# xguo7/SND-VAE

Hardware: AMD Instinct MI355X
Metric: training graphs/sec + ELBO-step ms, N=4096 d=64, at 1/2/4/8 MI355X (higher is better)
Workload: dtype bf16; 1 GPU; C2: node-latent SND-VAE train step, N=4096, d=64, 8 graphs/GPU, HIP-graph replay; n_nodes=4096, latent=64, graphs_per_gpu=8, global_batch=8, parallelism=dp1, hip_graph=True

## Files before the change

snd_vae_amd/csrc/snd_elem.hip:

```cpp
#include "snd_elem.hpp"

#include <algorithm>
#include "snd_gemm.hpp"
#include "snd_tref.hpp"

namespace snd {
namespace {

template <typename T>
__device__ __forceinline__ T block_sum(T v) {
  __shared__ T sh[16];
  v = (sizeof(T) == 8) ? (T)wave_sum_d((double)v) : (T)wave_sum((float)v);
  const int w = threadIdx.x >> 6, nw = blockDim.x >> 6;
  if ((threadIdx.x & 63) == 0) sh[w] = v;
  __syncthreads();
  T t = 0;
  if (threadIdx.x == 0)
    for (int k = 0; k < nw; ++k) t += sh[k];
  return t;
}

constexpr int kReparamGrid = 2048;

__global__ void __launch_bounds__(256) reparam_fwd_kernel(ReparamFwdArgs a) {
// ... 290 lines not shown
  }
  sg = lane_rows_sum<CP>(sg, red);
  sb = lane_rows_sum<CP>(sb, red);
  if (threadIdx.x < width) {
    const int stride = (a.has_enc ? 2 * a.wenc : 0) + 2 * a.h;
    float* pp = a.part + (long long)blockIdx.x * stride;
    int o = 0;
    if (a.has_enc) {
      pp[c] = sge * kBnC;
      pp[a.wenc + c] = sbe;
      o = 2 * a.wenc;
    }
    if (c < a.h) {
      pp[o + c] = sg * kBnC;
      pp[o + a.h + c] = sb;
    }
  }
}

#ifndef SND_RED_PL
#define SND_RED_PL 2
#endif
#ifndef SND_RED_PLS
#define SND_RED_PLS 4
#endif
#ifndef SND_RED_PLW
#define SND_RED_PLW 2
#endif
constexpr long long kRedWide = 2048;
__host__ __device__ __forceinline__ int red_pl(int nparts, long long items) {
  return nparts >= 1024 ? 64
                        : (nparts >= 256 ? 32 : (nparts >= 64 ? (items >= kRedWide ? SND_RED_PL : 8) : (items >= kRedWide ? SND_RED_PLW : SND_RED_PLS)));
}
struct ReducePack {
  ReduceDesc d[kMaxReduce];
  int bstart[kMaxReduce + 1];
};

template <int NTF> __device__ void finalize_block(const FinalizeArgs& a);

template <bool FIN, bool ADAM>
__global__ void __launch_bounds__(256) reduce_kernel(ReducePack pk, FinalizeArgs fin, ReduceAdam ra) {
  if constexpr (FIN) {
    if (blockIdx.x == 0) { finalize_block<256>(fin); return; }
  }
  const int bid = (int)blockIdx.x - (FIN ? 1 : 0);
  int di = 0;
#pragma unroll
  for (int i = 1; i < kMaxReduce; ++i) di += bid >= pk.bstart[i] ? 1 : 0;
  di = __builtin_amdgcn_readfirstlane(di);
  const ReduceDesc& d = pk.d[di];
  const int bx = bid - pk.bstart[di];
  const bool dad = ADAM && ((ra.mask >> di) & 1ull);
  float lrt = 0.f;
  if (dad) {
    const int st = *ra.stepn;
    lrt = (float)((double)ra.lr * sqrt(1.0 - pow((double)ra.b2, st)) / (1.0 - pow((double)ra.b1, st)));
  }
  __shared__ double red[256];
  const int rows = d.rows > 0 ? d.rows : 1;
  const long long items = (long long)rows * d.len;
  const int PL = red_pl(d.nparts, items);
  const int IPB = 256 / PL;
  const int it = threadIdx.x % IPB, pl = threadIdx.x / IPB;
  const long long j = (long long)bx * IPB + it;
  int r = 0, i = 0;
  double acc = 0.0;
  float pi = 0.f, mi = 0.f, vi = 0.f, prev = 0.f;
  if (j < items) {
    r = (int)(j / d.len);
    i = (int)(j - (long long)r * d.len);
    if (pl == 0) {
      const float* dst = d.dst + (long long)r * d.dst_rs + i;
      if (d.accumulate) prev = *dst;
      if constexpr (ADAM) {
        if (dad) {
          const long long k = dst - ra.gbase;
          pi = ra.p[k]; mi = ra.m[k]; vi = ra.v[k];
        }
      }
    }
    const float* src = d.src + (long long)r * d.src_rs + i;
    int p = pl;
    for (; p + 7 * PL < d.nparts; p += 8 * PL) {
      float v[8];
#pragma unroll
      for (int u = 0; u < 8; ++u) v[u] = src[(long long)(p + u * PL) * d.stride];
#pragma unroll
      for (int u = 0; u < 8; ++u) acc += (double)v[u];
    }
    for (; p + 3 * PL < d.nparts; p += 4 * PL) {
      const float v0 = src[(long long)p * d.stride];
      const float v1 = src[(long long)(p + PL) * d.stride];
      const float v2 = src[(long long)(p + 2 * PL) * d.stride];
      const float v3 = src[(long long)(p + 3 * PL) * d.stride];
      acc += (double)v0;
      acc += (double)v1;
      acc += (double)v2;
      acc += (double)v3;
    }
    for (; p < d.nparts; p += PL) acc += (double)src[(long long)p * d.stride];
  }
  red[threadIdx.x] = acc;
  __syncthreads();
  if (pl == 0 && j < items) {
    double t = 0.0;
    for (int q = 0; q < PL; ++q) t += red[q * IPB + it];
    float* dst = d.dst + (long long)r * d.dst_rs + i;
    float v = (float)(t * (double)d.scale);
    if (d.accumulate) v += prev;
    *dst = v;
    if constexpr (ADAM) {
      if (dad) {
        const long long k = dst - ra.gbase;
        adam_elem(pi, mi, vi, __fmul_rn(v, 1.f), ra.b1, ra.b2, ra.eps, lrt);
        ra.m[k] = mi;
// ... 145 lines not shown
  return 0;
}

int launch_enc_bwd(const EncBwdArgs& a, int rows, hipStream_t s) {
  const int width = a.has_enc ? a.wenc : a.h;
  if (width > 256) { set_error("enc_bwd: width %d > 256", width); return SND_ERR_ARG; }
  dim3 grid(col_blocks(rows));
  if (width <= 64) hipLaunchKernelGGL(enc_bwd_kernel<64>, grid, dim3(256), 0, s, a, rows);
  else if (width <= 128) hipLaunchKernelGGL(enc_bwd_kernel<128>, grid, dim3(256), 0, s, a, rows);
  else hipLaunchKernelGGL(enc_bwd_kernel<256>, grid, dim3(256), 0, s, a, rows);
  SND_LAUNCH_CHECK("enc_bwd_kernel");
  return 0;
}

int launch_reduce(const ReduceDesc* d, int n, hipStream_t s, const FinalizeArgs* fin,
                  const ReduceAdam* adam) {
  SND_CHECK_ARG(!adam || (n <= 64 && adam->gbase && adam->p && adam->m && adam->v && adam->stepn),
                "reduce: fused Adam needs <= 64 descriptors and its operands");
  for (int base = 0; base < n || (base == 0 && fin); base += kMaxReduce) {
    const bool last = base + kMaxReduce >= n;
    ReduceAdam ra{};
    if (adam) {
      ra = *adam;
      ra.mask = adam->mask >> base;
      if (n - base < 64) ra.mask &= (1ull << (n - base)) - 1;
    }
    const bool ad = ra.mask != 0;
    ReducePack pk{};
    const int cnt = n - base < kMaxReduce ? n - base : kMaxReduce;
    long long nb = 0;
    for (int i = 0; i < kMaxReduce; ++i) {
      pk.bstart[i] = (int)nb;
      if (i < cnt) {
        pk.d[i] = d[base + i];
        const long long items = (long long)(pk.d[i].rows > 0 ? pk.d[i].rows : 1) * pk.d[i].len;
        const int ipb = 256 / red_pl(pk.d[i].nparts, items);
        nb += (items + ipb - 1) / ipb;
      }
    }
    pk.bstart[kMaxReduce] = (int)nb;
    if (fin && last) {
      if (ad) hipLaunchKernelGGL((reduce_kernel<true, true>), dim3((unsigned)nb + 1), dim3(256), 0, s, pk, *fin, ra);
      else hipLaunchKernelGGL((reduce_kernel<true, false>), dim3((unsigned)nb + 1), dim3(256), 0, s, pk, *fin, ra);
    } else {
      if (nb == 0) continue;
      if (ad) hipLaunchKernelGGL((reduce_kernel<false, true>), dim3((unsigned)nb), dim3(256), 0, s, pk, FinalizeArgs{}, ra);
      else hipLaunchKernelGGL((reduce_kernel<false, false>), dim3((unsigned)nb), dim3(256), 0, s, pk, FinalizeArgs{}, ra);
    }
    SND_LAUNCH_CHECK("reduce_kernel");
  }
  return 0;
}

int launch_finalize(const FinalizeArgs& a, hipStream_t s) {
  hipLaunchKernelGGL(finalize_kernel, dim3(1), dim3(kFinT), 0, s, a);
  SND_LAUNCH_CHECK("finalize_kernel");
  return 0;
}

}

using namespace snd;

extern "C" int snd_reparam_kl_blocks(int rows, int latent) { return reparam_blocks(rows, latent); }
extern "C" int snd_sigmoid_mse_blocks(int rows) { return head_blocks(rows); }

extern "C" int snd_sigmoid_mse(const float* u, int ldu, int rows, int cin, const float* w,
// ... 64 lines not shown
```

snd_vae_amd/csrc/snd_fast.hip:

```cpp
#include "snd_fast.hpp"
#include "snd_gather.hpp"
#include "snd_pack.hpp"

#include <algorithm>

namespace snd {

namespace {

constexpr int NT = 256;

typedef short v4s __attribute__((ext_vector_type(4)));
typedef short v8s __attribute__((ext_vector_type(8)));
typedef __attribute__((address_space(3))) v4s lds_v4s;

__device__ __forceinline__ int swz(int row, int kp) {
  return kp >= 128 ? (row & 15) : (kp == 64 ? ((row >> 1) & 7) : 0);
}

__device__ __forceinline__ uint4 pack8(float4 lo, float4 hi) {
  bf16x8 v;
  v[0] = (__bf16)lo.x; v[1] = (__bf16)lo.y; v[2] = (__bf16)lo.z; v[3] = (__bf16)lo.w;
  v[4] = (__bf16)hi.x; v[5] = (__bf16)hi.y; v[6] = (__bf16)hi.z; v[7] = (__bf16)hi.w;
  return __builtin_bit_cast(uint4, v);
// ... 399 lines not shown
                                               int vlo, int vhi, int kp, __bf16* dst,
                                               const void* zero) {
  const int lane = threadIdx.x & 63, w = threadIdx.x >> 6;
  const int lk = log2kc(kp), kc = 1 << lk;
  const int npc = ((nrows << lk) + 63) >> 6;
  for (int j = w; j < npc; j += 4) {
    const int q = (j << 6) + lane;
    const int row = q >> lk, pc = q & (kc - 1);
    const int c = pc ^ trsw(row, kp);
    const int gr = base + row;
    const bool v = row < nrows && gr >= vlo && gr < vhi && 8 * c < K;
    const void* g = v ? (const void*)(src + (long long)gr * ld + 8 * c) : zero;
    glds16(g, reinterpret_cast<char*>(dst) + (j << 10));
  }
}

__device__ __forceinline__ int tr_off(int row, int col, int kp) {
  const int c = col >> 3;
  return row * kp + (((c ^ trsw(row, kp)) << 3) | (col & 4));
}

constexpr int WGT = 1024;

__device__ __forceinline__ int cdiv_d(int a, int b) { return (a + b - 1) / b; }

struct WgUnit { int sub, s0, s1, glo, ghi; };

__device__ __forceinline__ WgUnit wg_unit(const WgArgs& a, int sub, int s0, int c1) {
  const int send = min(c1, sub + kRcRows);
  WgUnit u;
  u.sub = sub; u.s0 = s0;
  if (a.T == 1) { u.glo = sub; u.ghi = send; u.s1 = send; }
  else {
    const int gs = (s0 / a.npg) * a.npg;
    u.glo = gs; u.ghi = min(a.R, gs + a.npg); u.s1 = min(send, u.ghi);
  }
  return u;
}

constexpr int kWgStampWords = 12;
__device__ __forceinline__ void wg_stamp(unsigned* ts, int i, bool on) {
  if (on && threadIdx.x == 0 && i < kWgStampWords) ts[i] = (unsigned)__builtin_amdgcn_s_memrealtime();
}

template <int NBO, int NPW = 1>
__device__ __forceinline__ void wgrad_body(const WgArgs& a, const int bx, const int by, __bf16* lds,
                                           unsigned* tsp = nullptr) {
  const bool stamp = tsp != nullptr;
  const int T = a.T, H = (T - 1) >> 1;
  const int XR = kRcRows + T - 1;
  const int kpx = a.K <= 32 ? 32 : (a.K <= 64 ? 64 : 128);
  const int kpy = a.N <= 32 ? 32 : (a.N <= 64 ? 64 : 128);
  const int xch = ((XR << log2kc(kpx)) + 63) & ~63;
  const int bufe = (xch << 3) + kRcRows * kpy;
  const int tid = threadIdx.x, lane = tid & 63, w = __builtin_amdgcn_readfirstlane(tid >> 6);
  const int li = lane & 15, lg = lane >> 4, tq = li >> 2, tp = li & 3;
  const __bf16* xg = reinterpret_cast<const __bf16*>(a.x);
  const __bf16* dg = reinterpret_cast<const __bf16*>(a.dy);
  const int c0 = bx * a.rows_per_wg, c1 = min(a.R, c0 + a.rows_per_wg);
  auto stage = [&](const WgUnit& u, int b) __attribute__((always_inline)) {
    if (kdbg(a.dbg) & 2) return;
    __bf16* xs = lds + b * bufe;
    __bf16* ds = xs + (xch << 3);
    const int lkx = log2kc(kpx), lky = log2kc(kpy);
    const int npx = xch >> 6, npy = (kRcRows << lky) >> 6;
    for (int j = w; j < npx + npy; j += WGT / 64) {
      const bool isx = j < npx;
      const int jj = isx ? j : j - npx;
      const int lk = isx ? lkx : lky, kp = isx ? kpx : kpy;
      const int q = (jj << 6) + lane;
      const int row = q >> lk, pc = q & ((1 << lk) - 1);
      const int c = pc ^ trsw(row, kp);
      const void* g = a.zero;
      if (isx) {
        const int gr = u.sub - H + row;
        if (row < XR && gr >= u.glo && gr < u.ghi && 8 * c < a.K) g = xg + (long long)gr * a.ldx + 8 * c;
      } else {
        const int gr = u.sub + row;
        if (gr >= u.s0 && gr < u.s1 && 8 * c < a.N) g = dg + (long long)gr * a.lddy + 8 * c;
      }
      glds16_async(g, reinterpret_cast<char*>(isx ? xs : ds) + (jj << 10));
    }
  };

  const WgUnit u0 = wg_unit(a, c0, c0, c1);
  if (c0 < c1) stage(u0, 0);
  const int cbn = (a.K + 15) >> 4;
  const int P = T * cbn;
  bool pvs[NPW];
  int ts[NPW], cbs[NPW];
#pragma unroll
  for (int i = 0; i < NPW; ++i) {
    const int wl = w + 16 * i, p = by * a.pairs_per_wg + wl;
    pvs[i] = wl < a.pairs_per_wg && p < P;
    ts[i] = pvs[i] ? p / cbn : 0;
    cbs[i] = pvs[i] ? p - ts[i] * cbn : 0;
  }
  const bool pv = pvs[0];

  f32x4 acc[NPW][NBO];
#pragma unroll
  for (int i = 0; i < NPW; ++i)
#pragma unroll
    for (int j = 0; j < NBO; ++j) acc[i][j] = f32x4{0.f, 0.f, 0.f, 0.f};

  const int rk0 = 8 * lg + tq;
  int xoff[NPW], xoff2[NPW];
#pragma unroll
  for (int i = 0; i < NPW; ++i) {
    xoff[i] = tr_off(rk0 + ts[i], 16 * cbs[i] + 4 * tp, kpx);
    xoff2[i] = tr_off(rk0 + ts[i] + 4, 16 * cbs[i] + 4 * tp, kpx);
  }
  if (kdbg(a.dbg) & 32) return;
  const int doff = rk0 * kpy;
  const int swd = trsw(rk0, kpy), tpl = (4 * tp) & 4, tph = tp >> 1;
  wg_stamp(tsp, 2, stamp);
  if (c0 < c1) {
    WgUnit u = u0;
    for (int k = 0;; ++k) {
      __builtin_amdgcn_s_waitcnt(0x0F70);
      __syncthreads();
      wg_stamp(tsp, 3 + k, stamp && k < 6);
      int nsub = u.sub, ns0 = u.s1;
      if (ns0 >= min(c1, u.sub + kRcRows)) { nsub = u.sub + kRcRows; ns0 = nsub; }
      const bool more = nsub < c1;
      WgUnit un{};
      if (more) { un = wg_unit(a, nsub, ns0, c1); stage(un, (k + 1) & 1); }
      const __bf16* xs = lds + (k & 1) * bufe;
      const __bf16* ds = xs + (xch << 3);
// ... 12 lines not shown
#pragma unroll
            for (int i = 0; i < NPW; ++i)
              if (i == 0 || pvs[i]) acc[i][ob] = __builtin_amdgcn_mfma_f32_16x16x32_bf16(af, bxv[i], acc[i][ob], 0, 0, 0);
          }
        }
      }
      if (!more) break;
      u = un;
    }
  }
  if (kdbg(a.dbg) & 8) return;
  const int sK = a.sK, sn4 = a.sn4;
#pragma unroll
  for (int i = 0; i < NPW; ++i) {
    const int k = 16 * cbs[i] + li;
    if (!pvs[i] || k >= a.K) continue;
    float* row = a.slab + (long long)bx * T * sK * sn4 + ((long long)ts[i] * sK + a.wk0 + k) * sn4 + a.wn0;
#pragma unroll
    for (int ob = 0; ob < NBO; ++ob) {
      const int n0 = 16 * ob + 4 * lg;
      if (n0 < a.N)
        *reinterpret_cast<float4*>(row + n0) =
            make_float4(acc[i][ob][0], acc[i][ob][1], acc[i][ob][2], acc[i][ob][3]);
    }
  }
}

template <int NBO>
__global__ void __launch_bounds__(WGT) wgrad_kernel(WgArgs a) {
  extern __shared__ __attribute__((aligned(16))) __bf16 lds[];
  wgrad_body<NBO>(a, blockIdx.x, blockIdx.y, lds);
}

struct WgMultiPack {
  WgArgs a[kMaxWgMulti];
  int start[kMaxWgMulti + 1];
  int nseg;
  int stamp_base;
};
static_assert(sizeof(WgMultiPack) <= 4096, "wgrad_multi: kernel arguments over 4 KB");

__global__ void __launch_bounds__(WGT) __attribute__((amdgpu_waves_per_eu(8, 8)))
wgrad_multi_kernel(WgMultiPack m) {
  extern __shared__ __attribute__((aligned(16))) __bf16 lds[];
  __shared__ unsigned tsl[kWgStampWords];
  const bool stamp = (kdbg(m.a[0].dbg) & (1 << 21)) && m.a[0].stamps;
  wg_stamp(tsl, 0, stamp);
  if (kdbg(m.a[0].dbg) & 1) return;
  const int bid = blockIdx.y * gridDim.x + blockIdx.x;
  int s = 0;
  if (gridDim.y > 1) {
    s = blockIdx.y;
  } else {
#pragma unroll
    for (int i = 1; i < kMaxWgMulti; ++i) s += (int)blockIdx.x >= m.start[i] ? 1 : 0;
  }
  s = __builtin_amdgcn_readfirstlane(s);
  const WgArgs a = m.a[s];
  const int local = gridDim.y > 1 ? (int)blockIdx.x : (int)blockIdx.x - m.start[s];
  const int gx = cdiv_d(a.R, a.rows_per_wg);
  const int bx = local % gx, by = local / gx;
  const bool two = a.pairs_per_wg > WGT / 64;
  if (kdbg(a.dbg) & 16) return;
  unsigned* ts = stamp ? tsl : nullptr;
  wg_stamp(ts, 1, stamp);
  switch ((a.N + 15) >> 4) {
    case 1: if (two) wgrad_body<1, 2>(a, bx, by, lds, ts); else wgrad_body<1>(a, bx, by, lds, ts); break;
    case 2: if (two) wgrad_body<2, 2>(a, bx, by, lds, ts); else wgrad_body<2>(a, bx, by, lds, ts); break;
    case 3: if (two) wgrad_body<3, 2>(a, bx, by, lds, ts); else wgrad_body<3>(a, bx, by, lds, ts); break;
    default: if (two) wgrad_body<4, 2>(a, bx, by, lds, ts); else wgrad_body<4>(a, bx, by, lds, ts); break;
  }
  if (stamp) {
    __syncthreads();
    if (threadIdx.x == 0) {
      unsigned* o = m.a[0].stamps + ((long long)m.stamp_base + bid) * kWgStampWords;
      for (int i = 0; i < 9; ++i) o[i] = tsl[i];
      o[9] = (unsigned)__builtin_amdgcn_s_memrealtime();
      o[10] = __builtin_amdgcn_s_getreg((31 << 11) | 4);
      o[11] = __builtin_amdgcn_s_getreg((31 << 11) | 20);
    }
  }
}

struct HeadFastPack { HeadFastArgs h[2]; };

template <int CIN, int COUT>
__device__ __forceinline__ void head_rows(const HeadFastArgs& h, int R) {
  constexpr int NQ = CIN * COUT + COUT + 3 * CIN;
  __shared__ float red[16][NQ];
  __shared__ double sred[4];
  const int tid = threadIdx.x, lane = tid & 63, w = tid >> 6;
  const int r = blockIdx.x * kHeadFastRows + tid;
  const bool rv = r < R;
  float wv[CIN][COUT], bv[COUT], gk[CIN], bk[CIN];
#pragma unroll
  for (int k = 0; k < CIN; ++k) {
#pragma unroll
    for (int o = 0; o < COUT; ++o) wv[k][o] = h.w[k * COUT + o];
    gk[k] = h.gamma[k] * kBnC;
    bk[k] = h.beta[k];
  }
#pragma unroll
  for (int o = 0; o < COUT; ++o) bv[o] = h.b[o];
  float u[CIN], yv[CIN];
#pragma unroll
  for (int k = 0; k < CIN; ++k) { u[k] = 0.f; yv[k] = 0.f; }
  if (rv) {
// ... 209 lines not shown
  SND_CHECK_ARG(a.ldx % 8 == 0 && a.ldo % 4 == 0, "rowconv: ldx %% 8 / ldo %% 4");
  a.npb = rc_cols_per_block(a.T, a.kp, a.np);
  SND_CHECK_ARG(a.npb > 0, "rowconv: LDS image too large (T %d kp %d np %d)", a.T, a.kp, a.np);
  for (;;) {
    const int nb = (int)round_up(cdiv(a.npb, 2), 16);
    if ((a.dbg & (1 << 19)) || a.g_rowptr || rc_blocks(a.R) * cdiv(a.np, a.npb) >= SND_RC_FILL || nb < 32 ||
        nb >= a.npb) break;
    a.npb = nb;
  }
  SND_CHECK_ARG(a.x && a.wpk && a.out && a.zero && a.x_bf16, "rowconv: null operand / fp32 x");
  SND_CHECK_ARG(!a.colpart || (a.ncp >= 1 && a.ncp <= 4), "rowconv: ncp");
  SND_CHECK_ARG(a.npg > 0, "rowconv: npg");
  SND_CHECK_ARG(!a.g_rowptr || (epi == RC_ENC0 && a.T == 1 && a.kp == 64 && a.K <= 64 && a.np <= 64 && a.g_colidx &&
                                a.gout && a.ldgo % 8 == 0 && a.ldx % 8 == 0 && a.npb == a.np),
                "rowconv: the gathered x rows need RC_ENC0, T 1, kp 64, one column window");
  switch (epi) {
    case RC_LIN: return rc_launch_epi<RC_LIN>(a, s);
    case RC_FWD:
      SND_CHECK_ARG(a.y && a.bias && a.gamma && a.beta && a.ldy % 4 == 0, "rowconv fwd: BN operands");
      return rc_launch_epi<RC_FWD>(a, s);
    case RC_DECBWD:
      SND_CHECK_ARG(a.y && a.gamma && a.beta && a.ldy % 4 == 0, "rowconv decbwd: BN operands");
      return rc_launch_epi<RC_DECBWD>(a, s);
    case RC_ENC1:
      SND_CHECK_ARG(a.p && a.xf && a.gamma && a.g2 && a.b2 && a.h % 4 == 0, "rowconv enc1 operands");
      return rc_launch_epi<RC_ENC1>(a, s);
    case RC_ENC0:
      SND_CHECK_ARG(a.p && a.w0 && a.gamma && a.f <= 4, "rowconv enc0 operands");
      return rc_launch_epi<RC_ENC0>(a, s);
    default: set_error("rowconv: bad epilogue %d", epi); return SND_ERR_ARG;
  }
}

static WgArgs wg_norm(const WgArgs& a) {
  WgArgs x = a;
  if (x.sK == 0) { x.sK = x.K; x.sn4 = wgrad_n4(x.N); x.wk0 = 0; x.wn0 = 0; }
  return x;
}

#ifndef SND_WG_SPLIT_LDS
#define SND_WG_SPLIT_LDS (80 * 1024)
#endif
constexpr size_t kWgSplitLds = SND_WG_SPLIT_LDS;
static int wg_split(const WgArgs& a, WgArgs* out, int cap) {
  const bool sk = a.K > 64 && wg_lds_bytes(a.T, a.K, std::min(a.N, 64)) > kWgSplitLds, sn = a.N > 64;
  int n = 0;
  for (int k0 = 0; k0 < a.K; k0 += sk ? 64 : a.K)
    for (int n0 = 0; n0 < a.N; n0 += sn ? 64 : a.N) {
      if (n >= cap) return -1;
      WgArgs w = a;
      w.K = sk ? std::min(64, a.K - k0) : a.K;
      w.N = sn ? std::min(64, a.N - n0) : a.N;
      w.x = static_cast<const __bf16*>(a.x) + k0;
      w.dy = static_cast<const __bf16*>(a.dy) + n0;
      w.wk0 = a.wk0 + k0; w.wn0 = a.wn0 + n0;
      w.pairs_per_wg = std::min(a.pairs_per_wg, a.T * cdiv(w.K, 16));
      out[n++] = w;
    }
  return n;
}

static int wg_multi_flush(WgMultiPack& pk, int total, size_t lds, hipStream_t s) {
  if (pk.nseg == 0) return 0;
  for (int i = pk.nseg; i <= kMaxWgMulti; ++i) pk.start[i] = total;
  bool uniform = pk.nseg > 1;
  for (int i = 1; i < pk.nseg; ++i) uniform = uniform && pk.start[i + 1] - pk.start[i] == pk.start[1];
  const dim3 grid = uniform ? dim3(pk.start[1], pk.nseg) : dim3(total);
  hipLaunchKernelGGL(wgrad_multi_kernel, grid, dim3(WGT), lds, s, pk);
  SND_LAUNCH_CHECK("wgrad_multi_kernel");
  return 0;
}

int launch_wgrad_multi(const WgArgs* a, int n, hipStream_t s) {
  if (n <= 0) return 0;
  WgMultiPack pk{};
  size_t lds = 0;
  int total = 0, base = 0;
  pk.nseg = 0;
  const bool stamps = a[0].stamps != nullptr;
  for (int i = 0; i < n; ++i) {
    const WgArgs x0 = wg_norm(a[i]);
    if (x0.R <= 0) continue;
    SND_CHECK_ARG(x0.T == 1 || x0.T == 5, "wgrad_multi: T must be 1 or 5");
    SND_CHECK_ARG(x0.K > 0 && x0.K <= 128 && x0.N > 0 && x0.N <= 128, "wgrad_multi: K %d N %d", x0.K, x0.N);
    SND_CHECK_ARG(x0.ldx % 8 == 0 && x0.lddy % 8 == 0 && x0.x_bf16 && x0.dy_bf16,
                  "wgrad_multi: bf16 operands with leading dims %% 8");
    SND_CHECK_ARG(x0.rows_per_wg % kRcRows == 0 && x0.pairs_per_wg >= 1 && x0.pairs_per_wg <= 2 * WGT / 64,
                  "wgrad_multi: geometry");
    SND_CHECK_ARG(x0.x && x0.dy && x0.slab && x0.zero && x0.npg > 0, "wgrad_multi: null operand");
    SND_CHECK_ARG(x0.sn4 % 4 == 0 && x0.wn0 % 4 == 0 && x0.wk0 + x0.K <= x0.sK &&
                  x0.wn0 + wgrad_n4(x0.N) <= x0.sn4, "wgrad_multi: slab window");
    WgArgs win[4];
    const int nw = wg_split(x0, win, 4);
    SND_CHECK_ARG(nw > 0, "wgrad_multi: window split");
    for (int j = 0; j < nw; ++j) {
      if (pk.nseg == kMaxWgMulti) {
        SND_TRY(wg_multi_flush(pk, total, lds, s));
        base += total;
        pk = WgMultiPack{};
        pk.stamp_base = base;
        lds = 0;
        total = 0;
      }
      const WgArgs& x = win[j];
      const int P = x.T * cdiv(x.K, 16);
      pk.a[pk.nseg] = x;
      pk.start[pk.nseg] = total;
      total += cdiv(x.R, x.rows_per_wg) * cdiv(P, x.pairs_per_wg);
      lds = std::max(lds, wg_lds_bytes(x.T, x.K, x.N));
      ++pk.nseg;
      SND_CHECK_ARG(!stamps || ((long long)base + total) * kWgStampWords <= a[0].stamp_words,
                    "wgrad_multi: %d workgroups' stamps exceed the %lld-word buffer", base + total,
                    a[0].stamp_words);
    }
  }
  return wg_multi_flush(pk, total, lds, s);
}

WgGeom wgrad_geom(int R, int T, int K, int N, int chunks) {
  WgGeom g{};
  const int P = T * cdiv(K, 16);
  g.pairs_per_wg = std::min(P, WGT / 64);
  g.gy = cdiv(P, g.pairs_per_wg);
  if (chunks > 0) {
    g.pairs_per_wg = std::min(P, 2 * WGT / 64);
    g.gy = cdiv(P, g.pairs_per_wg);
    g.rows_per_wg = (int)round_up(cdiv(R, chunks), kRcRows);
    g.gx = cdiv(R, g.rows_per_wg);
    return g;
  }
  int gx = std::max(1, 256 / g.gy);
  if ((long long)T * K * N >= 65536) gx = std::min(gx, 64);
  g.rows_per_wg = (int)round_up(cdiv(R, gx), kRcRows);
  g.gx = cdiv(R, g.rows_per_wg);
  return g;
}

int launch_wgrad(const WgArgs& a0, hipStream_t s) {
  const WgArgs a = wg_norm(a0);
  if (a.R <= 0) return 0;
  SND_CHECK_ARG(a.T == 1 || a.T == 5, "wgrad: T must be 1 or 5");
  SND_CHECK_ARG(a.K > 0 && a.K <= 128 && a.N > 0 && a.N <= 128, "wgrad: K %d N %d", a.K, a.N);
  SND_CHECK_ARG(a.ldx % 8 == 0 && a.lddy % 8 == 0 && a.x_bf16 && a.dy_bf16,
                "wgrad: bf16 operands with leading dims %% 8");
  SND_CHECK_ARG(a.rows_per_wg % kRcRows == 0 && a.pairs_per_wg >= 1 && a.pairs_per_wg <= WGT / 64,
                "wgrad: geometry");
  SND_CHECK_ARG(a.x && a.dy && a.slab && a.zero && a.npg > 0, "wgrad: null operand");
  const int P = a.T * cdiv(a.K, 16);
  dim3 grid(cdiv(a.R, a.rows_per_wg), cdiv(P, a.pairs_per_wg));
  switch (cdiv(a.N, 16)) {
    case 1: return wg_launch<1>(a, grid, s);
    case 2: return wg_launch<2>(a, grid, s);
    case 3: return wg_launch<3>(a, grid, s);
    case 4: return wg_launch<4>(a, grid, s);
    case 5: return wg_launch<5>(a, grid, s);
    case 6: return wg_launch<6>(a, grid, s);
    case 7: return wg_launch<7>(a, grid, s);
    default: return wg_launch<8>(a, grid, s);
  }
}

static thread_local int g_dbg = 0;
int debug_flags() { return g_dbg; }

static int fast_init_attributes_once() {
#define SND_ATTR(K)                                                                       \
  if (hipFuncSetAttribute(reinterpret_cast<const void*>(K),                               \
                          hipFuncAttributeMaxDynamicSharedMemorySize, (int)kMaxDynLds) != \
      hipSuccess) {                                                                       \
    set_error("hipFuncSetAttribute(%s) failed", #K);                                      \
    return SND_ERR_HIP;                                                                   \
  }
#define SND_ATTR4(E) SND_ATTR((rowconv_kernel<E, 1>)) SND_ATTR((rowconv_kernel<E, 2>)) \
                     SND_ATTR((rowconv_kernel<E, 3>)) SND_ATTR((rowconv_kernel<E, 4>))
  SND_ATTR4(RC_LIN) SND_ATTR4(RC_FWD) SND_ATTR4(RC_DECBWD) SND_ATTR4(RC_ENC1) SND_ATTR4(RC_ENC0)
#undef SND_ATTR4
  SND_ATTR((wgrad_kernel<1>)) SND_ATTR((wgrad_kernel<2>)) SND_ATTR((wgrad_kernel<3>))
  SND_ATTR((wgrad_kernel<4>)) SND_ATTR((wgrad_kernel<5>)) SND_ATTR((wgrad_kernel<6>))
  SND_ATTR((wgrad_kernel<7>)) SND_ATTR((wgrad_kernel<8>))
#undef SND_ATTR
  if (hipFuncSetAttribute(reinterpret_cast<const void*>(wgrad_multi_kernel),
                          hipFuncAttributeMaxDynamicSharedMemorySize, (int)kWgMultiLds) != hipSuccess) {
    set_error("hipFuncSetAttribute(wgrad_multi_kernel) failed");
    return SND_ERR_HIP;
  }
  return 0;
}

int fast_init_attributes() {
  static const int rc = fast_init_attributes_once();
  return rc;
}

}

extern "C" int snd_debug_set(int flags) {
  snd::g_dbg = flags;
  return 0;
}
```

snd_vae_amd/csrc/snd_fast.hpp:

```cpp
#pragma once
#include "snd_common.hpp"

namespace snd {

struct ColMap {
  int a, b, offb;
  __host__ __device__ int phys() const { return b ? offb + b : a; }
  __host__ __device__ bool valid(int c) const { return c < a || (b && c >= offb && c < offb + b); }
  __host__ __device__ int logical(int c) const { return c < a ? c : c - offb + a; }
};
inline ColMap colmap_plain(int n) { return {n, 0, n}; }
inline ColMap colmap_split(int a, int b) { return {a, b, (int)round_up(a, 8)}; }

struct PackSrc {
  const float* w;
  int A, B;
  int a0, a1, b0, b1;
  int n_off, k_off;
  int mode;
};
struct PackDesc {
  __bf16* dst;
  int T, kp, np;
  int nsrc;
  PackSrc s[2];
};
constexpr int kMaxPack = 16;
int launch_pack(const PackDesc* d, int n, hipStream_t s);
size_t pack_bytes(int T, int kp, int np);

enum RcEpi {
  RC_LIN = 0,
  RC_FWD = 1,
// ... 1 lines not shown
  RC_ENC1 = 3,
  RC_ENC0 = 4,
};
struct RcArgs {
  const void* x; int ldx; int K; int x_bf16;
  int R, npg, T;
  const __bf16* wpk; int kp, np;
  int N;
  ColMap cols;
  const float* bias; const float* gamma; const float* beta;
  const float* bias_b; const float* gamma_b; const float* beta_b;
  float* y; int ldy;
  void* out; int ldo; int out_bf16;
  float* colpart; int ncp;
  const float* p; int ldp;
  const float* xf; int ldxf; int f;
  const float* w0;
  const float* g2; const float* b2;
  int h;
  const void* zero;
  int dbg;
  int ktail; const float* wtail; int ldwt;
  int npb;
  const int* g_rowptr; const int* g_colidx; void* gout; int ldgo;
};
constexpr int kRcRows = 128;
constexpr size_t kRcLdsLimit = 136 * 1024;
int rc_blocks(int R);
size_t rc_lds_bytes(int T, int kp, int np);
int rc_cols_per_block(int T, int kp, int np);
int launch_rowconv(const RcArgs& a, int epi, hipStream_t s);

struct WgArgs {
  const void* x; int ldx; int K; int x_bf16;
  const void* dy; int lddy; int N; int dy_bf16;
  int R, npg, T;
  int rows_per_wg;
  int pairs_per_wg;
  float* slab;
  const void* zero;
  int dbg;
  int sK, sn4, wk0, wn0;
  unsigned* stamps;
  long long stamp_words;
};
struct WgGeom { int rows_per_wg, pairs_per_wg, gx, gy; };
WgGeom wgrad_geom(int R, int T, int K, int N, int chunks = 0);
inline int wgrad_n4(int N) { return (N + 3) & ~3; }
int launch_wgrad(const WgArgs& a, hipStream_t s);
constexpr int kMaxWgMulti = 32;
int launch_wgrad_multi(const WgArgs* a, int n, hipStream_t s);

struct HeadFastArgs {
  const void* u; int ldu; int u_bf16;
  const float* y; int ldy;
  const float* gamma; const float* beta;
  int cin;
  const float* w; const float* b; int cout;
  const float* target; int ldt;
  float count;
  float* yhat;
  __bf16* dy; int lddy;
  float* part;
  double* sse;
};
constexpr int kHeadFastRows = 256;
int heads_fast_blocks(int R);
bool heads_fast_supported(int cin, int cout);
int heads_fast_parts(int cin, int cout);
int launch_heads_fast(const HeadFastArgs* h, int n, int R, hipStream_t s);

struct Gcn0Args {
  const int* rowptr; const int* colidx; int R;
  const float* x; int ldx; int f;
  const float* w0; const float* g0; const float* b0; int h0;
  __bf16* h1; int ldh1;
  float* ax; __bf16* axb;
  int xcd_nbg;
  const int* row_order;
  PackDesc pack[kMaxPack]; int pack_blk[kMaxPack + 1]; int npack;
};
int xcd_nbg(int npg, int ngraphs);
int gcn0_blocks(int R);
int launch_gcn0(const Gcn0Args& a, hipStream_t s);
// ... 61 lines not shown
```

snd_vae_amd/csrc/snd_step.hip:

```cpp
#include <algorithm>
#include <cstdarg>
#include <cstdlib>
#include <cstring>
#include <new>
#include <string>
#include <vector>

#include "snd_dec.hpp"
#include "snd_decode.hpp"
#include "snd_elem.hpp"
#include "snd_fast.hpp"
#include "snd_gemm.hpp"
#include "snd_head.hpp"
#include "snd_spmm.hpp"
#include "snd_tref.hpp"
#include "snd_sg.hpp"
#include "snd_zzt.hpp"

namespace snd {

static thread_local char g_err[512] = "";

void set_error(const char* fmt, ...) {
  va_list ap;
// ... 1374 lines not shown
                 p.c.h1, SND_SPMM_PLAIN, (__bf16*)(ws + p.buf("FDXW1")), p.c.h1};
    a.xcd_nbg = xcd_nbg(p.N, p.B);
    use_tiles(a, batch, p.N, p.B);
    return launch_spmm_bf16(a, s);
  }
  if (!strncmp(kernel, "tref_", 5)) {
    SND_CHECK_ARG(p.tref && !p.sg && p.last_params, "snd_plan_launch: no graph-latent step has run");
    Ctx x{&p, ws, p.last_params, p.last_grads, s};
    const snd_config_t& c = p.c;
    const long long KH = (long long)p.N * p.W, CP = (long long)p.N * p.dj;
    const float adj_scale = (float)(2.0 * (double)c.norm / ((double)p.B * p.N * (double)p.N));
    const __bf16* gb = p.fast_enc ? reinterpret_cast<const __bf16*>(x.f("FG")) : nullptr;
    if (!strcmp(kernel, "tref_head_fwd")) {
      TrefHeadFwdArgs a{gb ? nullptr : x.f("G"), KH, p.B, x.w("enc.Wh"), c.g_hidden, x.w("enc.bh"),
                        x.f("PHF"), gb, p.ldg, p.W, p.N};
      return launch_tref_head_fwd(a, s);
    }
    if (!strcmp(kernel, "tref_head_bwd")) {
      TrefHeadBwdArgs a{gb ? nullptr : x.f("G"), KH, p.B, x.w("enc.Wh"), c.g_hidden, x.f("DH"),
                        x.g("enc.Wh"), gb ? nullptr : x.f("DG"), gb, p.ldg, p.W, p.N,
                        gb ? reinterpret_cast<__bf16*>(x.f("FDG")) : nullptr};
      return launch_tref_head_bwd(a, s);
    }
    if (!strcmp(kernel, "tref_proj_fwd")) {
      TrefProjFwdArgs a{x.f("ZL"), p.B, c.latent, x.w("dec.Wp"), x.w("dec.bp"), CP, x.f("Z")};
      return launch_tref_proj_fwd(a, s);
    }
    if (!strcmp(kernel, "tref_proj_bwd")) {
      TrefProjBwdArgs a{x.f("ZL"), p.B, c.latent, x.w("dec.Wp"), CP, x.f("DZDEC"), x.f("DJD"), x.f("EJ"),
                        adj_scale, x.g("dec.Wp"), x.g("dec.bp"), x.f("PDZ")};
      return launch_tref_proj_bwd(a, s);
    }
  }
  if (!strcmp(kernel, "wgrad_multi")) {
    SND_CHECK_ARG(!p.last_wq.empty(), "snd_plan_launch: no multi-segment weight-gradient launch yet");
    std::vector<WgArgs> q = p.last_wq;
    for (auto& w : q) {
      w.dbg = debug_flags();
      const bool st = (w.dbg & (1 << 21)) && p.dec_fused;
      w.stamps = st ? reinterpret_cast<unsigned*>(ws + p.buf("PDHS")) : nullptr;
      w.stamp_words = st ? p.buf_numel("PDHS") : 0;
    }
    return launch_wgrad_multi(q.data(), (int)q.size(), s);
  }
  if (!strcmp(kernel, "head_bwd")) {
    SND_CHECK_ARG(p.head_bwd && p.last_params, "snd_plan_launch: head_bwd needs a fused-head step first");
    Ctx x{&p, ws, p.last_params, p.last_grads, s};
    x.zts = p.last_zts;
    const double pairs = (double)p.B * p.N * (double)p.N;
    return head_bwd_fused(x, batch, (float)(2.0 * (double)p.c.norm / pairs),
                          (float)((double)p.c.beta / ((double)p.RH * p.c.latent)));
  }
  if (!strcmp(kernel, "head_fwd")) {
    SND_CHECK_ARG(p.head_fused && p.last_params, "snd_plan_launch: head_fwd needs a fused-head step first");
    Ctx x{&p, ws, p.last_params, p.last_grads, s};
    const ZztStage stg = zzt_stage(ws + p.buf("ZSTAGE"), p.B, p.N, p.dj, p.c.dtype);
    return head_fwd_fused(x, batch, nullptr, 0ull, nullptr, stg);
  }
  if (!strncmp(kernel, "dec:", 4) || !strcmp(kernel, "pack")) {
    SND_CHECK_ARG(p.fast && p.last_params, "snd_plan_launch: no fast-path step has run");
    SND_TRY(fast_init_attributes());
    Ctx x{&p, ws, p.last_params, p.last_grads, s};
    if (kernel[0] == 'p') return pack_decoder(x);
    if (!strcmp(kernel, "dec:fwd") || !strcmp(kernel, "dec:bwd")) {
      SND_CHECK_ARG(p.dec_fused, "snd_plan_launch: %s needs the fused decoder", kernel);
      return decoder_fast(x, batch, kernel[4] == 'f' ? 100 : 101);
    }
    return decoder_fast(x, batch, atoi(kernel + 4));
  }
  set_error("snd_plan_launch: unknown kernel '%s'", kernel);
  return SND_ERR_ARG;
}

void final_reduce_descs(const Ctx& x, std::vector<ReduceDesc>& rd) {
// ... 405 lines not shown
```

Baseline: 39340 graphs/s.

## Cut scalar prologue cost in reduce and wgrad_multi kernels via vector argument loads

The reduce kernel now reads the block-start table as three 16-dword vectors, stores each segment's base block inside a 64-byte aligned descriptor, and issues the first R0 strided loads early so they overlap the Adam bias-correction pow/sqrt. The wgrad_multi kernel reorders WgArgs so a 16-dword header loads in one go, precomputes gx, a packed geometry word and a magic reciprocal for npg on the host, and replaces integer divisions with compares or a multiply-high. Uniform packs now launch a 3D grid selected by a template flag, and a dims query entry point is added. The goal is to shorten kernel prologues, which are dominated by scalar loads and divisions. The cost is extra register pressure from the early loads and a new limit of at most 3 pair groups per segment.

```diff
diff --git a/snd_vae_amd/csrc/snd_elem.hip b/snd_vae_amd/csrc/snd_elem.hip
--- a/snd_vae_amd/csrc/snd_elem.hip
+++ b/snd_vae_amd/csrc/snd_elem.hip
@@ -346,10 +346,29 @@
   return nparts >= 1024 ? 64
                         : (nparts >= 256 ? 32 : (nparts >= 64 ? (items >= kRedWide ? SND_RED_PL : 8) : (items >= kRedWide ? SND_RED_PLW : SND_RED_PLS)));
 }
+struct alignas(64) RedSeg {
+  const float* src;
+  float* dst;
+  int nparts;
+  int len;
+  long long stride;
+  float scale;
+  int accumulate;
+  int rows;
+  int b0;
+  long long src_rs, dst_rs;
+};
+static_assert(sizeof(RedSeg) == 64, "RedSeg: one 16-dword load");
 struct ReducePack {
-  ReduceDesc d[kMaxReduce];
+  RedSeg d[kMaxReduce];
   int bstart[kMaxReduce + 1];
 };
+static_assert(kMaxReduce == 48 && offsetof(ReducePack, bstart) % 64 == 0, "bstart is read as three 16-dword vectors");
+typedef int red_i16_t __attribute__((ext_vector_type(16)));
+
+#ifndef SND_RED_R0
+#define SND_RED_R0 8
+#endif
 
 template <int NTF> __device__ void finalize_block(const FinalizeArgs& a);
 
@@ -358,19 +377,27 @@
   if constexpr (FIN) {
     if (blockIdx.x == 0) { finalize_block<256>(fin); return; }
   }
-  const int bid = (int)blockIdx.x - (FIN ? 1 : 0);
+  int bid = (int)blockIdx.x - (FIN ? 1 : 0);
+  const red_i16_t s0 = *reinterpret_cast<const red_i16_t*>(&pk.bstart[0]);
+  const red_i16_t s1 = *reinterpret_cast<const red_i16_t*>(&pk.bstart[16]);
+  const red_i16_t s2 = *reinterpret_cast<const red_i16_t*>(&pk.bstart[32]);
+  if constexpr (ADAM)
+    asm("" : "+s"(bid) : "s"(s0), "s"(s1), "s"(s2), "s"(ra.mask), "s"(ra.gbase), "s"(ra.p), "s"(ra.m), "s"(ra.v),
+        "s"(ra.stepn));
+  else
+    asm("" : "+s"(bid) : "s"(s0), "s"(s1), "s"(s2));
   int di = 0;
 #pragma unroll
-  for (int i = 1; i < kMaxReduce; ++i) di += bid >= pk.bstart[i] ? 1 : 0;
+  for (int i = 1; i < kMaxReduce; ++i) di = bid >= (i < 16 ? s0[i] : (i < 32 ? s1[i - 16] : s2[i - 32])) ? i : di;
   di = __builtin_amdgcn_readfirstlane(di);
-  const ReduceDesc& d = pk.d[di];
-  const int bx = bid - pk.bstart[di];
+  const RedSeg d = pk.d[di];
+  int st = 0;
+  if constexpr (ADAM) st = *ra.stepn;
+  int b0 = d.b0;
+  asm("" : "+s"(b0) : "s"(d.src), "s"(d.dst), "s"(d.nparts), "s"(d.len), "s"(d.stride), "s"(d.scale),
+      "s"(d.accumulate), "s"(d.rows), "s"(d.src_rs), "s"(d.dst_rs), "s"(st));
+  const int bx = bid - b0;
   const bool dad = ADAM && ((ra.mask >> di) & 1ull);
-  float lrt = 0.f;
-  if (dad) {
-    const int st = *ra.stepn;
-    lrt = (float)((double)ra.lr * sqrt(1.0 - pow((double)ra.b2, st)) / (1.0 - pow((double)ra.b1, st)));
-  }
   __shared__ double red[256];
   const int rows = d.rows > 0 ? d.rows : 1;
   const long long items = (long long)rows * d.len;
@@ -381,9 +408,16 @@
   int r = 0, i = 0;
   double acc = 0.0;
   float pi = 0.f, mi = 0.f, vi = 0.f, prev = 0.f;
+  constexpr int R0 = SND_RED_R0;
+  float v0[R0];
+#pragma unroll
+  for (int u = 0; u < R0; ++u) v0[u] = 0.f;
+  const float* src = d.src;
+  const bool ld0 = j < items && d.nparts > 0;
   if (j < items) {
-    r = (int)(j / d.len);
-    i = (int)(j - (long long)r * d.len);
+    if (rows == 1) { r = 0; i = (int)j; }
+    else if (items < (1ll << 31)) { r = (int)((unsigned)j / (unsigned)d.len); i = (int)((unsigned)j - (unsigned)r * (unsigned)d.len); }
+    else { r = (int)(j / d.len); i = (int)(j - (long long)r * d.len); }
     if (pl == 0) {
       const float* dst = d.dst + (long long)r * d.dst_rs + i;
       if (d.accumulate) prev = *dst;
@@ -394,8 +428,21 @@
         }
       }
     }
-    const float* src = d.src + (long long)r * d.src_rs + i;
-    int p = pl;
+    src = d.src + (long long)r * d.src_rs + i;
+  }
+  if (ld0) {
+#pragma unroll
+    for (int u = 0; u < R0; ++u) v0[u] = src[(long long)min(pl + u * PL, d.nparts - 1) * d.stride];
+  }
+  asm volatile("" ::: "memory");
+  float lrt = 0.f;
+  if (dad) lrt = (float)((double)ra.lr * sqrt(1.0 - pow((double)ra.b2, st)) / (1.0 - pow((double)ra.b1, st)));
+  asm volatile("" : "+v"(lrt) :: "memory");
+  if (j < items) {
+#pragma unroll
+    for (int u = 0; u < R0; ++u)
+      if (pl + u * PL < d.nparts) acc += (double)v0[u];
+    int p = pl + R0 * PL;
     for (; p + 7 * PL < d.nparts; p += 8 * PL) {
       float v[8];
 #pragma unroll
@@ -607,7 +654,9 @@
     for (int i = 0; i < kMaxReduce; ++i) {
       pk.bstart[i] = (int)nb;
       if (i < cnt) {
-        pk.d[i] = d[base + i];
+        const ReduceDesc& x = d[base + i];
+        pk.d[i] = RedSeg{x.src, x.dst, x.nparts, x.len, x.stride, x.scale, x.accumulate, x.rows, (int)nb,
+                         x.src_rs, x.dst_rs};
         const long long items = (long long)(pk.d[i].rows > 0 ? pk.d[i].rows : 1) * pk.d[i].len;
         const int ipb = 256 / red_pl(pk.d[i].nparts, items);
         nb += (items + ipb - 1) / ipb;
diff --git a/snd_vae_amd/csrc/snd_fast.hip b/snd_vae_amd/csrc/snd_fast.hip
--- a/snd_vae_amd/csrc/snd_fast.hip
+++ b/snd_vae_amd/csrc/snd_fast.hip
@@ -455,7 +455,8 @@
   u.sub = sub; u.s0 = s0;
   if (a.T == 1) { u.glo = sub; u.ghi = send; u.s1 = send; }
   else {
-    const int gs = (s0 / a.npg) * a.npg;
+    const int g = a.npg_m ? (int)(((unsigned long long)(unsigned)s0 * a.npg_m) >> 32) : s0 / a.npg;
+    const int gs = g * a.npg;
     u.glo = gs; u.ghi = min(a.R, gs + a.npg); u.s1 = min(send, u.ghi);
   }
   return u;
@@ -508,16 +509,17 @@
 
   const WgUnit u0 = wg_unit(a, c0, c0, c1);
   if (c0 < c1) stage(u0, 0);
-  const int cbn = (a.K + 15) >> 4;
+  const int cbn = a.geo & 255, ppw = a.geo >> 8;
   const int P = T * cbn;
   bool pvs[NPW];
   int ts[NPW], cbs[NPW];
 #pragma unroll
   for (int i = 0; i < NPW; ++i) {
-    const int wl = w + 16 * i, p = by * a.pairs_per_wg + wl;
-    pvs[i] = wl < a.pairs_per_wg && p < P;
-    ts[i] = pvs[i] ? p / cbn : 0;
-    cbs[i] = pvs[i] ? p - ts[i] * cbn : 0;
+    const int wl = w + 16 * i, p = by * ppw + wl;
+    pvs[i] = wl < ppw && p < P;
+    const int t = (p >= cbn) + (p >= 2 * cbn) + (p >= 3 * cbn) + (p >= 4 * cbn);
+    ts[i] = pvs[i] ? t : 0;
+    cbs[i] = pvs[i] ? p - t * cbn : 0;
   }
   const bool pv = pvs[0];
 
@@ -596,14 +598,17 @@
   wgrad_body<NBO>(a, blockIdx.x, blockIdx.y, lds);
 }
 
-struct WgMultiPack {
-  WgArgs a[kMaxWgMulti];
+struct alignas(64) WgMultiPack {
   int start[kMaxWgMulti + 1];
   int nseg;
   int stamp_base;
+  WgArgs a[kMaxWgMulti];
 };
 static_assert(sizeof(WgMultiPack) <= 4096, "wgrad_multi: kernel arguments over 4 KB");
 
+typedef int wg_hdr_t __attribute__((ext_vector_type(16), aligned(8)));
+typedef int wg_i16_t __attribute__((ext_vector_type(16)));
+template <bool G3>
 __global__ void __launch_bounds__(WGT) __attribute__((amdgpu_waves_per_eu(8, 8)))
 wgrad_multi_kernel(WgMultiPack m) {
   extern __shared__ __attribute__((aligned(16))) __bf16 lds[];
@@ -611,20 +616,37 @@
   const bool stamp = (kdbg(m.a[0].dbg) & (1 << 21)) && m.a[0].stamps;
   wg_stamp(tsl, 0, stamp);
   if (kdbg(m.a[0].dbg) & 1) return;
-  const int bid = blockIdx.y * gridDim.x + blockIdx.x;
-  int s = 0;
-  if (gridDim.y > 1) {
-    s = blockIdx.y;
+  int s = 0, first = 0;
+  if constexpr (G3) {
+    s = blockIdx.z;
   } else {
-#pragma unroll
-    for (int i = 1; i < kMaxWgMulti; ++i) s += (int)blockIdx.x >= m.start[i] ? 1 : 0;
-  }
-  s = __builtin_amdgcn_readfirstlane(s);
-  const WgArgs a = m.a[s];
-  const int local = gridDim.y > 1 ? (int)blockIdx.x : (int)blockIdx.x - m.start[s];
-  const int gx = cdiv_d(a.R, a.rows_per_wg);
-  const int bx = local % gx, by = local / gx;
-  const bool two = a.pairs_per_wg > WGT / 64;
+    static_assert(kMaxWgMulti == 32, "start[] is read as two 16-dword vectors");
+    const wg_i16_t lo = *reinterpret_cast<const wg_i16_t*>(&m.start[0]);
+    const wg_i16_t hi = *reinterpret_cast<const wg_i16_t*>(&m.start[16]);
+    asm volatile("" :: "s"(lo), "s"(hi));
+#pragma unroll
+    for (int i = 1; i < kMaxWgMulti; ++i) {
+      const int st = i < 16 ? lo[i] : hi[i - 16];
+      const bool in = (int)blockIdx.x >= st;
+      s = in ? i : s;
+      first = in ? st : first;
+    }
+    s = __builtin_amdgcn_readfirstlane(s);
+    first = __builtin_amdgcn_readfirstlane(first);
+  }
+  WgArgs a = m.a[s];
+  const wg_hdr_t hdr = *reinterpret_cast<const wg_hdr_t*>(&m.a[s]);
+  __builtin_memcpy(&a, &hdr, sizeof(hdr));
+  asm volatile("" :: "s"(a.slab), "s"(a.sK), "s"(a.sn4), "s"(a.wk0), "s"(a.wn0), "s"(a.geo));
+  int bx, by;
+  if constexpr (G3) {
+    bx = blockIdx.x; by = blockIdx.y;
+  } else {
+    const int local = (int)blockIdx.x - first;
+    by = (local >= a.gx) + (local >= 2 * a.gx);
+    bx = local - by * a.gx;
+  }
+  const bool two = (a.geo >> 8) > WGT / 64;
   if (kdbg(a.dbg) & 16) return;
   unsigned* ts = stamp ? tsl : nullptr;
   wg_stamp(ts, 1, stamp);
@@ -637,6 +659,7 @@
   if (stamp) {
     __syncthreads();
     if (threadIdx.x == 0) {
+      const int bid = (G3 ? m.start[s] : first) + by * a.gx + bx;
       unsigned* o = m.a[0].stamps + ((long long)m.stamp_base + bid) * kWgStampWords;
       for (int i = 0; i < 9; ++i) o[i] = tsl[i];
       o[9] = (unsigned)__builtin_amdgcn_s_memrealtime();
@@ -912,9 +935,15 @@
   }
 }
 
+static void wg_quotients(WgArgs& x) {
+  x.gx = x.rows_per_wg > 0 ? cdiv(x.R, x.rows_per_wg) : 0;
+  x.geo = cdiv(x.K, 16) | (x.pairs_per_wg << 8);
+  x.npg_m = (x.npg >= 2 && (long long)x.R * x.npg < (1ll << 32)) ? (unsigned)((1ull << 32) / (unsigned)x.npg) + 1u : 0u;
+}
 static WgArgs wg_norm(const WgArgs& a) {
   WgArgs x = a;
   if (x.sK == 0) { x.sK = x.K; x.sn4 = wgrad_n4(x.N); x.wk0 = 0; x.wn0 = 0; }
+  wg_quotients(x);
   return x;
 }
 
@@ -935,24 +964,30 @@
       w.dy = static_cast<const __bf16*>(a.dy) + n0;
       w.wk0 = a.wk0 + k0; w.wn0 = a.wn0 + n0;
       w.pairs_per_wg = std::min(a.pairs_per_wg, a.T * cdiv(w.K, 16));
+      wg_quotients(w);
       out[n++] = w;
     }
   return n;
 }
 
-static int wg_multi_flush(WgMultiPack& pk, int total, size_t lds, hipStream_t s) {
+static int wg_gy(const WgArgs& x) { return cdiv(x.T * cdiv(x.K, 16), x.pairs_per_wg); }
+
+static int wg_multi_flush(WgMultiPack& pk, int total, size_t lds, hipStream_t s, int* dims) {
   if (pk.nseg == 0) return 0;
   for (int i = pk.nseg; i <= kMaxWgMulti; ++i) pk.start[i] = total;
-  bool uniform = pk.nseg > 1;
-  for (int i = 1; i < pk.nseg; ++i) uniform = uniform && pk.start[i + 1] - pk.start[i] == pk.start[1];
-  const dim3 grid = uniform ? dim3(pk.start[1], pk.nseg) : dim3(total);
-  hipLaunchKernelGGL(wgrad_multi_kernel, grid, dim3(WGT), lds, s, pk);
+  const int gx = pk.a[0].gx, gy = wg_gy(pk.a[0]);
+  bool uniform = pk.nseg > 1 && !((unsigned)debug_flags() & (1u << 31));
+  for (int i = 1; i < pk.nseg; ++i) uniform = uniform && pk.a[i].gx == gx && wg_gy(pk.a[i]) == gy;
+  if (dims) { *dims = std::min(*dims, uniform ? 3 : 1); return 0; }
+  if (uniform) hipLaunchKernelGGL(wgrad_multi_kernel<true>, dim3(gx, gy, pk.nseg), dim3(WGT), lds, s, pk);
+  else hipLaunchKernelGGL(wgrad_multi_kernel<false>, dim3(total), dim3(WGT), lds, s, pk);
   SND_LAUNCH_CHECK("wgrad_multi_kernel");
   return 0;
 }
 
-int launch_wgrad_multi(const WgArgs* a, int n, hipStream_t s) {
+int launch_wgrad_multi(const WgArgs* a, int n, hipStream_t s, int* dims) {
   if (n <= 0) return 0;
+  if (dims) *dims = 3;
   WgMultiPack pk{};
   size_t lds = 0;
   int total = 0, base = 0;
@@ -965,7 +1000,8 @@
     SND_CHECK_ARG(x0.K > 0 && x0.K <= 128 && x0.N > 0 && x0.N <= 128, "wgrad_multi: K %d N %d", x0.K, x0.N);
     SND_CHECK_ARG(x0.ldx % 8 == 0 && x0.lddy % 8 == 0 && x0.x_bf16 && x0.dy_bf16,
                   "wgrad_multi: bf16 operands with leading dims %% 8");
-    SND_CHECK_ARG(x0.rows_per_wg % kRcRows == 0 && x0.pairs_per_wg >= 1 && x0.pairs_per_wg <= 2 * WGT / 64,
+    SND_CHECK_ARG(x0.rows_per_wg % kRcRows == 0 && x0.rows_per_wg > 0 && x0.pairs_per_wg >= 1 &&
+                      x0.pairs_per_wg <= 2 * WGT / 64,
                   "wgrad_multi: geometry");
     SND_CHECK_ARG(x0.x && x0.dy && x0.slab && x0.zero && x0.npg > 0, "wgrad_multi: null operand");
     SND_CHECK_ARG(x0.sn4 % 4 == 0 && x0.wn0 % 4 == 0 && x0.wk0 + x0.K <= x0.sK &&
@@ -975,7 +1011,7 @@
     SND_CHECK_ARG(nw > 0, "wgrad_multi: window split");
     for (int j = 0; j < nw; ++j) {
       if (pk.nseg == kMaxWgMulti) {
-        SND_TRY(wg_multi_flush(pk, total, lds, s));
+        SND_TRY(wg_multi_flush(pk, total, lds, s, dims));
         base += total;
         pk = WgMultiPack{};
         pk.stamp_base = base;
@@ -983,10 +1019,10 @@
         total = 0;
       }
       const WgArgs& x = win[j];
-      const int P = x.T * cdiv(x.K, 16);
+      SND_CHECK_ARG(wg_gy(x) <= 3, "wgrad_multi: %d pair groups", wg_gy(x));
       pk.a[pk.nseg] = x;
       pk.start[pk.nseg] = total;
-      total += cdiv(x.R, x.rows_per_wg) * cdiv(P, x.pairs_per_wg);
+      total += x.gx * wg_gy(x);
       lds = std::max(lds, wg_lds_bytes(x.T, x.K, x.N));
       ++pk.nseg;
       SND_CHECK_ARG(!stamps || ((long long)base + total) * kWgStampWords <= a[0].stamp_words,
@@ -994,7 +1030,7 @@
                     a[0].stamp_words);
     }
   }
-  return wg_multi_flush(pk, total, lds, s);
+  return wg_multi_flush(pk, total, lds, s, dims);
 }
 
 WgGeom wgrad_geom(int R, int T, int K, int N, int chunks) {
@@ -1017,8 +1053,9 @@
 }
 
 int launch_wgrad(const WgArgs& a0, hipStream_t s) {
-  const WgArgs a = wg_norm(a0);
+  WgArgs a = wg_norm(a0);
   if (a.R <= 0) return 0;
+  if (a.pairs_per_wg > WGT / 64) { a.pairs_per_wg = WGT / 64; wg_quotients(a); }
   SND_CHECK_ARG(a.T == 1 || a.T == 5, "wgrad: T must be 1 or 5");
   SND_CHECK_ARG(a.K > 0 && a.K <= 128 && a.N > 0 && a.N <= 128, "wgrad: K %d N %d", a.K, a.N);
   SND_CHECK_ARG(a.ldx % 8 == 0 && a.lddy % 8 == 0 && a.x_bf16 && a.dy_bf16,
@@ -1059,7 +1096,9 @@
   SND_ATTR((wgrad_kernel<4>)) SND_ATTR((wgrad_kernel<5>)) SND_ATTR((wgrad_kernel<6>))
   SND_ATTR((wgrad_kernel<7>)) SND_ATTR((wgrad_kernel<8>))
 #undef SND_ATTR
-  if (hipFuncSetAttribute(reinterpret_cast<const void*>(wgrad_multi_kernel),
+  if (hipFuncSetAttribute(reinterpret_cast<const void*>(wgrad_multi_kernel<true>),
+                          hipFuncAttributeMaxDynamicSharedMemorySize, (int)kWgMultiLds) != hipSuccess ||
+      hipFuncSetAttribute(reinterpret_cast<const void*>(wgrad_multi_kernel<false>),
                           hipFuncAttributeMaxDynamicSharedMemorySize, (int)kWgMultiLds) != hipSuccess) {
     set_error("hipFuncSetAttribute(wgrad_multi_kernel) failed");
     return SND_ERR_HIP;
diff --git a/snd_vae_amd/csrc/snd_fast.hpp b/snd_vae_amd/csrc/snd_fast.hpp
--- a/snd_vae_amd/csrc/snd_fast.hpp
+++ b/snd_vae_amd/csrc/snd_fast.hpp
@@ -1,4 +1,5 @@
 #pragma once
+#include <cstddef>
 #include "snd_common.hpp"
 
 namespace snd {
@@ -66,24 +67,28 @@
 int launch_rowconv(const RcArgs& a, int epi, hipStream_t s);
 
 struct WgArgs {
-  const void* x; int ldx; int K; int x_bf16;
-  const void* dy; int lddy; int N; int dy_bf16;
-  int R, npg, T;
+  const void* x; const void* dy;
+  const void* zero;
+  int R, ldx, lddy, K, N, T, npg;
   int rows_per_wg;
+  int geo;
+  unsigned npg_m;
+  float* slab;
+  int sK, sn4, wk0, wn0;
+  int gx;
   int pairs_per_wg;
-  float* slab;
-  const void* zero;
   int dbg;
-  int sK, sn4, wk0, wn0;
+  short x_bf16, dy_bf16;
   unsigned* stamps;
   long long stamp_words;
 };
+static_assert(offsetof(WgArgs, slab) == 64 && sizeof(WgArgs) == 120, "WgArgs: the 16-dword header; 120 bytes");
 struct WgGeom { int rows_per_wg, pairs_per_wg, gx, gy; };
 WgGeom wgrad_geom(int R, int T, int K, int N, int chunks = 0);
 inline int wgrad_n4(int N) { return (N + 3) & ~3; }
 int launch_wgrad(const WgArgs& a, hipStream_t s);
 constexpr int kMaxWgMulti = 32;
-int launch_wgrad_multi(const WgArgs* a, int n, hipStream_t s);
+int launch_wgrad_multi(const WgArgs* a, int n, hipStream_t s, int* dims = nullptr);
 
 struct HeadFastArgs {
   const void* u; int ldu; int u_bf16;
diff --git a/snd_vae_amd/csrc/snd_step.hip b/snd_vae_amd/csrc/snd_step.hip
--- a/snd_vae_amd/csrc/snd_step.hip
+++ b/snd_vae_amd/csrc/snd_step.hip
@@ -1430,7 +1430,8 @@
       return launch_tref_proj_bwd(a, s);
     }
   }
-  if (!strcmp(kernel, "wgrad_multi")) {
+  const bool wg_dims = !strcmp(kernel, "wgrad_multi:dims");
+  if (wg_dims || !strcmp(kernel, "wgrad_multi")) {
     SND_CHECK_ARG(!p.last_wq.empty(), "snd_plan_launch: no multi-segment weight-gradient launch yet");
     std::vector<WgArgs> q = p.last_wq;
     for (auto& w : q) {
@@ -1438,6 +1439,11 @@
       const bool st = (w.dbg & (1 << 21)) && p.dec_fused;
       w.stamps = st ? reinterpret_cast<unsigned*>(ws + p.buf("PDHS")) : nullptr;
       w.stamp_words = st ? p.buf_numel("PDHS") : 0;
+    }
+    if (wg_dims) {
+      int dims = 0;
+      SND_TRY(launch_wgrad_multi(q.data(), (int)q.size(), s, &dims));
+      return dims;
     }
     return launch_wgrad_multi(q.data(), (int)q.size(), s);
   }
```

After: 39790 graphs/s, median of 6. 1.1% higher.
